# audeering/opensmile

Measured on NVIDIA H100. Metric: LLD frames/sec (16kHz, 25ms/10ms), higher is better.
Workload: dtype f32

## Files before the change

opensmile_b200/csrc/lld_common.cuh:

```cuda
#pragma once
#include <cstdio>

#include "fft_radix.cuh"
#include "kernels.cuh"

namespace osm {

struct SmemLayout {
  int zbuf, samp, raw, rawPcm, mbar, winLut, tw, splitTw, melCoef, melRange, dctCos, dctLift, eql, melS, ring;
  int total;
  int sampFloats, rawPcmBytes;
};

__host__ __device__ inline int align_up(int x, int a) { return (x + a - 1) / a * a; }

constexpr int kLeadFrames = 8;

__host__ __device__ inline SmemLayout make_layout(const LldParams &p, int M, int F)
{
  SmemLayout L;
  int o = 0;
  L.zbuf = o; o += M * F * 8;
  const int S = p.frameStep + p.sPad;
  L.sampFloats = align_up((F - 1) * S + p.frameSize + ((p.frameSize - 1) / p.frameStep) * p.sPad + 2, 4);
  L.samp = o; o += L.sampFloats * 4;
  L.raw = o; o += F * 4;
  o = align_up(o, 16);
  L.rawPcmBytes = align_up(16 + (kLeadFrames + (F - 1) * p.frameStep + p.frameSize) * p.nChan * 2, 16);
  L.rawPcm = o; o += L.rawPcmBytes;
  L.mbar = o; o += 16;
  L.winLut = o; o += M * 16;
  L.tw = o; o += p.twCount * 8;
  L.splitTw = o; o += (M / 2 + 1) * 8;
  o = align_up(o, 16);
  L.melCoef = o; o += (p.melVCount + 4) * 8;
  L.melRange = o; o += 2 * (p.nBands + 2) * 4;
  o = align_up(o, 16);
  L.dctCos = o; o += max(p.dctRows * p.dctStride, p.opKind == 0 ? p.nBands * 16 : 0) * 4;
  L.dctLift = o; o += p.nStat * 4;
  L.eql = o; o += (p.opKind == 1 ? p.nBands : 0) * 4;
  o = align_up(o, 16);
  if (L.sampFloats >= p.nBands * F) L.melS = L.samp;
  else { L.melS = o; o += p.nBands * F * 4; }
  L.ring = o; o += p.nStat * 2 * F * 4;
  L.total = align_up(o, 16);
  return L;
}

__device__ __forceinline__ float div32767(float x)
{
  const float rc = 3.0518509447574615e-05f;
  const float q0 = __fmul_rn(x, rc);
  const float r = __fmaf_rn(-q0, 32767.0f, x);
  return __fmaf_rn(r, rc, q0);
}

#define OSM_COLD __noinline__
template <bool F32>
__device__ __forceinline__ float pcm_to_float_generic(const int16_t *s, int nChan)
{
  if constexpr (F32) return *reinterpret_cast<const float *>(s);
  float tmp = (float)s[0];
  for (int c = 1; c < nChan; c++) tmp = __fadd_rn(tmp, (float)s[c]);
  if (nChan == 1) return div32767(tmp);
  if (nChan == 2) return div32767(tmp * 0.5f);
  return __fdiv_rn(__fdiv_rn(tmp, (float)nChan), 32767.0f);
}
template <bool F32>
static __device__ OSM_COLD float pcm_to_float_slow(const int16_t *s, int nChan) { return pcm_to_float_generic<F32>(s, nChan); }

__device__ __forceinline__ uint32_t smem_u32(const void *p) { return (uint32_t)__cvta_generic_to_shared(p); }

__device__ __forceinline__ void mbar_init(uint64_t *bar, int count)
{
  asm volatile("mbarrier.init.shared::cta.b64 [%0], %1;" ::"r"(smem_u32(bar)), "r"(count));
  asm volatile("fence.mbarrier_init.release.cluster;" ::: "memory");
}
__device__ __forceinline__ void mbar_expect_tx(uint64_t *bar, uint32_t bytes)
{
  asm volatile("mbarrier.arrive.expect_tx.shared::cta.b64 _, [%0], %1;" ::"r"(smem_u32(bar)), "r"(bytes) : "memory");
}
__device__ __forceinline__ void bulk_g2s(void *dst, const void *src, uint32_t bytes, uint64_t *bar)
{
  asm volatile("cp.async.bulk.shared::cluster.global.mbarrier::complete_tx::bytes [%0], [%1], %2, [%3];"
               ::"r"(smem_u32(dst)), "l"(src), "r"(bytes), "r"(smem_u32(bar)) : "memory");
}
__device__ __forceinline__ void mbar_wait(uint64_t *bar, uint32_t parity)
{
  asm volatile(
      "{\n"
      ".reg .pred p;\n"
      "LAB_WAIT:\n"
      "mbarrier.try_wait.parity.shared::cta.b64 p, [%0], %1;\n"
      "@p bra LAB_DONE;\n"
      "bra LAB_WAIT;\n"
      "LAB_DONE:\n"
      "}\n" ::"r"(smem_u32(bar)), "r"(parity) : "memory");
}

struct ChunkCtx {
  int utt, a, b;
  int T;
  int s0;
  int sEnd;
  int nT;
  int tile0;
  long long uo;
  long long row0;
};

template <int F>
__device__ __forceinline__ ChunkCtx load_chunk(const LldParams &p, int chunk)
{
  ChunkCtx c;
  const ChunkRef cr = p.chunks[chunk];
  c.utt = cr.utt; c.a = cr.a; c.b = cr.b; c.tile0 = cr.tile0;
  c.uo = p.uttOff[cr.utt];
  const long long Ls = p.uttOff[cr.utt + 1] - c.uo;
  c.T = (int)((Ls - p.frameSize) / p.frameStep + 1);
  c.s0 = max(cr.a - p.halo, 0);
  c.sEnd = min(cr.b + p.halo, c.T);
  c.nT = (c.sEnd - c.s0 + F - 1) / F;
  c.row0 = p.rowOff[cr.utt];
  return c;
}

__device__ __forceinline__ int chunk_run_begin(const LldParams &p, int g)
{
  const long long w = (long long)p.chunks[0].w0 + (long long)g * p.ctaTiles;
  int lo = 0, hi = p.nChunks;
  while (lo < hi) {
    const int mid = (lo + hi) >> 1;
    if (p.chunks[mid].w0 < w) lo = mid + 1;
    else hi = mid;
  }
  return lo;
}

struct TileGeom {
  int fs;
  int nf;
  int count;
  int lead;
  int mis;
  uint32_t bytes;
  const char *src;
};

template <int F>
__device__ __forceinline__ TileGeom tile_geom(const LldParams &p, const ChunkCtx &c, int j)
{
  TileGeom g;
  g.fs = c.s0 + j * F;
  g.nf = min(F, c.sEnd - g.fs);
  const long long s0 = (long long)g.fs * p.frameStep;
  g.count = (g.nf - 1) * p.frameStep + p.frameSize;
  g.lead = (s0 > 0) ? kLeadFrames : 0;
  const char *a = reinterpret_cast<const char *>(p.pcm + (c.uo + s0 - g.lead) * p.nChan);
  g.mis = (int)(reinterpret_cast<uintptr_t>(a) & 15);
  g.src = a - g.mis;
  g.bytes = (uint32_t)align_up(g.mis + (g.lead + g.count) * p.nChan * 2, 16);
  return g;
}

__device__ __forceinline__ float div_exact(float x, float d, float rcp)
{
  const float ax = fabsf(x);
  if (rcp != 0.f && ax > 1e-30f && ax < 1e30f) {
    const float q0 = __fmul_rn(x, rcp);
    const float r = __fmaf_rn(-q0, d, x);
    return __fmaf_rn(r, rcp, q0);
  }
  return __fdiv_rn(x, d);
}

__device__ __forceinline__ int win_navail(int t, int n0, int c0, int Tprev)
{
  return (t < c0) ? Tprev : min(n0 + (t - c0) + 1, Tprev);
}

template <int M, int F, int NVW, int R, int MS, bool FIRST, bool LAST, bool VEC2>
__device__ __forceinline__ void fft_stage(float2 *__restrict__ Z, const float *__restrict__ sampF,
                                          const float *__restrict__ raw,
                                          const float4 *__restrict__ winLut,
                                          const float2 *__restrict__ tw,
                                          const LldParams &p, int vw, int f)
{
  constexpr int stride = MS / R;
  for (int t = vw; t < M / R; t += NVW) {
    const int blk = t / stride, j = t % stride;
    const int base = blk * MS + j;
    float2 v[R];
    if (FIRST) {
#pragma unroll
      for (int r = 0; r < R; r++) {
        const float4 wl = winLut[base + stride * r];
        const int off = __float_as_int(wl.z);
        float2 x;
        if (VEC2) {
          x = *reinterpret_cast<const float2 *>(sampF + off);
        } else {
          x.x = sampF[off];
          x.y = sampF[off + 1];
        }
        v[r] = make_float2(__fmul_rn(x.x, wl.x), __fmul_rn(x.y, wl.y));
      }
      if (base == 0 && p.preemph)
        v[0].x = __fmul_rn(__fmul_rn(p.oneMinusK, raw[f]), winLut[0].x);
      if (p.hasWinOffset) {
#pragma unroll
        for (int r = 0; r < R; r++) {
          const float nv = winLut[base + stride * r].w;
          if (nv >= 1.f) v[r].x = __fadd_rn(v[r].x, p.winOffset);
          if (nv >= 2.f) v[r].y = __fadd_rn(v[r].y, p.winOffset);
        }
      }
    } else {
#pragma unroll
      for (int r = 0; r < R; r++) v[r] = Z[(base + stride * r) * F + f];
    }
    Dft<R>::run(v);
    if (!LAST) {
      const float2 *twj = tw + j * R;
#pragma unroll
      for (int q = 1; q < R; q++) v[Dft<R>::out(q)] = cmul(v[Dft<R>::out(q)], twj[q]);
    }
#pragma unroll
    for (int q = 0; q < R; q++) Z[(base + stride * q) * F + f] = v[Dft<R>::out(q)];
  }
}

constexpr int kMaxLp = 8;

template <int F, int NVW>
__device__ __forceinline__ void plp_backend(const LldParams &p, const float *melS, const float *sCos,
                                            const float *sLift, float *acfS, float *dst, int vw, int f)
{
  const int nB = p.nBands, nFreq = p.plpNFreq, nAuto = p.plpNAuto;
  if (!p.plpIDFT) {
    for (int i = vw; i < nB; i += NVW) dst[i * (2 * F) + f] = melS[i * F + f];
    return;
  }
  for (int i = vw; i < nAuto; i += NVW) {
    const float *ct = sCos + i * p.dctStride;
    double tmp = 0.0;
    if (p.plpHtk) tmp = (double)ct[0] * (double)melS[f];
    for (int m = 1; m < nFreq - 1; m++) tmp = __dadd_rn(tmp, (double)ct[m] * (double)melS[(m - 1) * F + f]);
    tmp = __dadd_rn(tmp, (double)ct[nFreq - 1] * (double)melS[(nFreq - 3) * F + f]);
    const float a = (float)(tmp / (2.0 * (double)(nFreq - 1)));
    if (!p.plpLP) dst[i * (2 * F) + f] = a;
    else acfS[i * F + f] = a;
  }
  if (!p.plpLP) return;
  __syncthreads();
  if (vw == 0) {
    const int P = p.plpOrder;
    float r[kMaxLp + 1], a[kMaxLp], cc[kMaxLp + 1];
#pragma unroll
    for (int i = 0; i <= kMaxLp; i++) r[i] = (i <= P) ? acfS[i * F + f] : 0.f;
#pragma unroll
    for (int i = 0; i < kMaxLp; i++) a[i] = 0.f;
    float gain = 0.f;
    if (r[0] != 0.f) {
      float e = r[0];
#pragma unroll
      for (int m = 1; m <= kMaxLp; m++) {
        if (m <= P && e != 0.f) {
          float sum = r[m];
#pragma unroll
          for (int i = 1; i < m; i++) sum = __fadd_rn(sum, __fmul_rn(a[i - 1], r[m - i]));
          const float km = __fmul_rn(__fdiv_rn(-1.0f, e), sum);
          a[m - 1] = km;
#pragma unroll
          for (int i = 1; i <= m / 2; i++) {
            const float x = a[i - 1];
            a[i - 1] = __fadd_rn(a[i - 1], __fmul_rn(km, a[m - i - 1]));
            if ((i < (m / 2)) || ((m & 1) == 1)) a[m - i - 1] = __fadd_rn(a[m - i - 1], __fmul_rn(km, x));
          }
          e = __fmul_rn(e, __fsub_rn(1.0f, __fmul_rn(km, km)));
        }
      }
      gain = e;
    }
    if (!p.plpCeps) {
#pragma unroll
      for (int i = 0; i < kMaxLp; i++) if (i < P) dst[i * (2 * F) + f] = a[i];
      return;
    }
    if (gain <= 0.f) gain = 1.0f;
    int first = p.plpFirstCC < 1 ? 1 : p.plpFirstCC;
    const int last = p.plpLastCC > P ? P : p.plpLastCC;
#pragma unroll
    for (int n = 1; n <= kMaxLp; n++) {
      if (n >= first && n <= last) {
        double sum = 0.0;
#pragma unroll
        for (int i = 1; i < n; i++)
          sum = __dadd_rn(sum, (double)__fmul_rn(__fmul_rn((float)(n - i), a[i - 1]), cc[n - i - 1]));
        cc[n - first] = -__fadd_rn(a[n - first], (float)(sum / (double)n));
      }
    }
    const float zeroth = (float)(-log(1.0 / (double)gain));
    const int nC = p.nStat;
#pragma unroll
    for (int i = 0; i <= kMaxLp; i++) {
      if (i < nC) {
        float v;
        if (p.plpFirstCC == 0) {
          if (p.plpHtk) v = (i == nC - 1) ? zeroth : cc[i];
          else v = (i == 0) ? zeroth : cc[i - 1];
        } else {
          v = cc[i];
        }
        if (p.plpLifter) v = __fmul_rn(v, sLift[i]);
        dst[i * (2 * F) + f] = v;
      }
    }
  }
}

template <int F, int NT>
__device__ __forceinline__ void emit_interior(const float *__restrict__ ring, float *__restrict__ Dbuf,
                                              float *__restrict__ outS, int K, int dRows, int slot0, int rslot0,
                                              float norm1, float rcp1, float norm2, float rcp2, int tid)
{
  const int K3 = 3 * K;
  constexpr int DR = F + 4;
  for (int item = tid; item < K * DR; item += NT) {
    const int c = item / DR, tt = item - c * DR;
    const float *rc = ring + c * (2 * F);
    const int sl = slot0 + tt;
    const float dA = __fsub_rn(rc[(sl + 1) & (2 * F - 1)], rc[(sl - 1) & (2 * F - 1)]);
    const float dB = __fsub_rn(rc[(sl + 2) & (2 * F - 1)], rc[(sl - 2) & (2 * F - 1)]);
    const float dv = div_exact(__fadd_rn(dA, __fmul_rn(2.0f, dB)), norm1, rcp1);
    Dbuf[c * dRows + tt] = dv;
    const int rr = tt - 2;
    if (rr >= 0 && rr < F) outS[rr * K3 + K + c] = dv;
  }
  for (int item = tid; item < K * F; item += NT) {
    const int c = item / F, rr = item - c * F;
    outS[rr * K3 + c] = ring[c * (2 * F) + ((rslot0 + rr) & (2 * F - 1))];
  }
  __syncthreads();
  for (int item = tid; item < K * F; item += NT) {
    const int c = item / F, rr = item - c * F;
    const float *dt = Dbuf + c * dRows + rr + 2;
    const float dA = __fsub_rn(dt[1], dt[-1]);
    const float dB = __fsub_rn(dt[2], dt[-2]);
    outS[rr * K3 + 2 * K + c] = div_exact(__fadd_rn(dA, __fmul_rn(2.0f, dB)), norm2, rcp2);
  }
  __syncthreads();
}

template <int F, int NW>
__device__ OSM_COLD void emit_edge(const float *__restrict__ ring, float *__restrict__ Dbuf, float *__restrict__ outS,
                               int K, int W1, int W2, int T, int T1, int c01, int c02, int s0, int r0, int r1,
                               int d0, int d1, int dRows, float norm1, float rcp1, float norm2, float rcp2,
                               int warp, int lane)
{
  const int K3 = 3 * K, nr = r1 - r0;
  for (int c = warp; c < K; c += NW) {
    const float *rc = ring + c * (2 * F);
    for (int tt = lane; tt < d1 - d0; tt += 32) {
      const int t = d0 + tt;
      float num = 0.f;
      for (int i = 1; i <= W1; i++) {
        const int hi = t + i, lo = t - i;
        float later, prior;
        if (t - W1 < 0) {
          later = (hi >= T) ? 0.f : rc[(hi - s0) & (2 * F - 1)];
          prior = rc[(max(lo, 0) - s0) & (2 * F - 1)];
        } else {
          later = rc[(min(hi, T - 1) - s0) & (2 * F - 1)];
          prior = rc[(min(lo, T - 1) - s0) & (2 * F - 1)];
        }
        num = __fadd_rn(num, __fmul_rn((float)i, __fsub_rn(later, prior)));
      }
      const float dv = div_exact(num, norm1, rcp1);
      Dbuf[c * dRows + tt] = dv;
      if (t >= r0 && t < r1) outS[(t - r0) * K3 + K + c] = dv;
    }
    for (int rr = lane; rr < nr; rr += 32) outS[rr * K3 + c] = rc[(r0 + rr - s0) & (2 * F - 1)];
  }
  __syncthreads();
  for (int c = warp; c < K; c += NW) {
    const float *dc = Dbuf + c * dRows - d0;
    for (int rr = lane; rr < nr; rr += 32) {
      const int t = r0 + rr;
      const int navail2 = win_navail(t, c01, c02, T1);
      float num = 0.f;
      for (int i = 1; i <= W2; i++) {
        const int hi = t + i, lo = t - i;
        float later, prior;
        if (t - W2 < 0) {
          later = (hi >= navail2) ? 0.f : dc[hi];
          prior = dc[max(lo, 0)];
        } else {
          later = dc[min(hi, navail2 - 1)];
          prior = dc[min(lo, navail2 - 1)];
        }
        num = __fadd_rn(num, __fmul_rn((float)i, __fsub_rn(later, prior)));
      }
      outS[rr * K3 + 2 * K + c] = div_exact(num, norm2, rcp2);
    }
  }
  __syncthreads();
}

}
```

opensmile_b200/csrc/lld_fast.cu:

```cuda
#include "lld_common.cuh"

namespace osm {

enum { kPhStage, kPhPass1, kPhPass2, kPhMel, kPhDct, kPhEmit, kPhStore, kPhKernel, kPhKernelMax, kPhTiles, kPhSlots };
#ifdef OSM_LLD_PHASE_CLOCKS
__device__ unsigned long long gLld512Phase[kPhSlots];
#define OSM_PHASE(k)                                                    \
  do {                                                                  \
    if (tid == 0) {                                                     \
      const long long c_ = clock64();                                   \
      sPh[k] += (unsigned long long)(c_ - phT);                         \
      phT = c_;                                                         \
    }                                                                   \
  } while (0)
#else
#define OSM_PHASE(k) do {} while (0)
#endif

namespace {

constexpr int kM = 256, kF = 32, kNT = 256, kNW = 8;
constexpr int kKMax = 16;
constexpr int kPartOff = 9216;

__device__ __forceinline__ void dft4_d0(float2 &a, float2 &b, float2 &c, float2 &d)
{
  const float2 t0 = cadd(a, c), t1 = csub(a, c), bb = b;
  a = cadd(t0, bb);
  c = csub(t0, bb);
  b = make_float2(t1.x + bb.y, t1.y - bb.x);
  d = make_float2(t1.x - bb.y, t1.y + bb.x);
}

template <int NZR>
__device__ __forceinline__ void dft16_first(float2 (&v)[16])
{
  dft4(v[0], v[4], v[8], v[12]);
  if (NZR <= 13) {
    dft4_d0(v[1], v[5], v[9], v[13]);
    dft4_d0(v[2], v[6], v[10], v[14]);
    dft4_d0(v[3], v[7], v[11], v[15]);
  } else {
    dft4(v[1], v[5], v[9], v[13]);
    dft4(v[2], v[6], v[10], v[14]);
    dft4(v[3], v[7], v[11], v[15]);
  }
  const float c1 = 0.92387953251128675613f, s1 = 0.38268343236508977173f;
  const float c2 = 0.70710678118654752440f;
  v[5] = cmul(v[5], make_float2(c1, -s1));
  { float2 a = v[6]; v[6] = make_float2(c2 * (a.x + a.y), c2 * (a.y - a.x)); }
  v[7] = cmul(v[7], make_float2(s1, -c1));
  { float2 a = v[9]; v[9] = make_float2(c2 * (a.x + a.y), c2 * (a.y - a.x)); }
  v[10] = cmul_mi(v[10]);
  { float2 a = v[11]; v[11] = make_float2(c2 * (a.y - a.x), -c2 * (a.x + a.y)); }
  v[13] = cmul(v[13], make_float2(s1, -c1));
  { float2 a = v[14]; v[14] = make_float2(c2 * (a.y - a.x), -c2 * (a.x + a.y)); }
  v[15] = cmul(v[15], make_float2(-c1, s1));
#pragma unroll
  for (int k1 = 0; k1 < 4; k1++) dft4(v[4 * k1], v[4 * k1 + 1], v[4 * k1 + 2], v[4 * k1 + 3]);
}

__device__ __forceinline__ void split_pair(float2 a, float2 b, float2 w, float &pk, float &pm)
{
  const float2 e2 = make_float2(a.x + b.x, a.y - b.y);
  const float2 o2 = make_float2(a.x - b.x, a.y + b.y);
  const float2 t2 = cmul(o2, w);
  const float xr = e2.x + t2.y, xi = e2.y - t2.x;
  const float yr = e2.x - t2.y, yi = e2.y + t2.x;
  pk = __fmaf_rn(xr, xr, __fmul_rn(xi, xi));
  pm = __fmaf_rn(yr, yr, __fmul_rn(yi, yi));
}

template <int NZR>
__global__ void __launch_bounds__(kNT, 2) lld512_kernel(const LldParams p)
{
  constexpr int M = kM, F = kF, NT = kNT, NW = kNW;
  using D16 = Dft<16>;

  extern __shared__ __align__(16) unsigned char smem[];
  __shared__ ChunkCtx sCx[2];
  __shared__ int sRun[2];
  const SmemLayout L = make_layout(p, M, F);
  float2 *Z = reinterpret_cast<float2 *>(smem + L.zbuf);
  float *P = reinterpret_cast<float *>(smem + L.zbuf);
  float *samp = reinterpret_cast<float *>(smem + L.samp);
  float *raw = reinterpret_cast<float *>(smem + L.raw);
  unsigned char *rawPcm = smem + L.rawPcm;
  uint64_t *mbar = reinterpret_cast<uint64_t *>(smem + L.mbar);
  float4 *sWinLut = reinterpret_cast<float4 *>(smem + L.winLut);
  float2 *sTw = reinterpret_cast<float2 *>(smem + L.tw);
  float2 *sSplit = reinterpret_cast<float2 *>(smem + L.splitTw);
  float2 *sMelCoef = reinterpret_cast<float2 *>(smem + L.melCoef);
  int *sMelRange = reinterpret_cast<int *>(smem + L.melRange);
  float *sDct = reinterpret_cast<float *>(smem + L.dctCos);
  float *sLift = reinterpret_cast<float *>(smem + L.dctLift);
  float *ring = reinterpret_cast<float *>(smem + L.ring);
  float *Dbuf = reinterpret_cast<float *>(smem + L.zbuf);

  const int tid = threadIdx.x;
  const int warp = tid >> 5, f = tid & 31;

  if (tid == 0) mbar_init(mbar, 1);
  if (tid < 2) sRun[tid] = chunk_run_begin(p, blockIdx.x + tid);
  for (int i = tid; i < M; i += NT) sWinLut[i] = p.winLut[i];
  for (int i = tid; i < p.twCount; i += NT) sTw[i] = p.twiddles[i];
  for (int i = tid; i < M / 2 + 1; i += NT) sSplit[i] = p.splitTw[i];
  for (int i = tid; i < p.melVCount; i += NT) sMelCoef[i] = p.melVisit[i];
  for (int i = tid; i < p.nBands + 2; i += NT) { sMelRange[i] = p.melRange[i]; sMelRange[p.nBands + 2 + i] = p.melVB[i]; }
  for (int i = tid; i < p.nBands * kKMax; i += NT) {
    const int m = i / kKMax, c = i - m * kKMax;
    sDct[i] = (c < p.nStat) ? p.dctCos[c * p.dctStride + m] : 0.f;
  }
  for (int i = tid; i < p.nStat; i += NT) sLift[i] = p.dctLift[i];
  for (int i = tid; i < L.sampFloats; i += NT) samp[i] = 0.f;
  for (int i = tid; i < F; i += NT) raw[i] = 0.f;
  __syncthreads();

  const int hop = p.frameStep;
  const int S = hop + p.sPad;
  uint32_t phase = 0;
#ifdef OSM_LLD_PHASE_CLOCKS
  __shared__ unsigned long long sPh[kPhSlots];
  if (tid < kPhSlots) sPh[tid] = 0;
  const long long phT0 = clock64();
  long long phT = phT0;
#endif

  int chunk = sRun[0];
  const int chunkEnd = sRun[1];
  if (chunk >= chunkEnd) return;
  int cpar = 0;
  if (tid == 0) {
    sCx[0] = load_chunk<F>(p, chunk);
    const TileGeom g0 = tile_geom<F>(p, sCx[0], 0);
    mbar_expect_tx(mbar, g0.bytes);
    bulk_g2s(rawPcm, g0.src, g0.bytes, mbar);
  }
  __syncthreads();
  int j = 0;
  int emitted = sCx[0].a;

  const int tA = (warp == 0) ? 0 : warp, tB = (warp == 0) ? 8 : 16 - warp;
  const int wl = (warp == 0) ? 8 : warp, wh = (warp == 0) ? 0 : warp;
  const int melBs = p.melSplit[warp], melBe = p.melSplit[warp + 1];

  while (chunk < chunkEnd) {
    const ChunkCtx &cx = sCx[cpar];

    mbar_wait(mbar, phase);
    phase ^= 1;
    {
      const TileGeom tg = tile_geom<F>(p, cx, j);
      const int count = tg.count;
      const int16_t *rp = reinterpret_cast<const int16_t *>(rawPcm + tg.mis) + tg.lead;
      const bool aligned = (tg.mis == 0);
      const bool hasLead = tg.lead > 0;
      const float ks = p.preDe ? p.preK : -p.preK;
#pragma unroll 1
      for (int i = tid * 8; i < count; i += NT * 8) {
        int wds[4];
        if (aligned) {
          const int4 w4 = *reinterpret_cast<const int4 *>(rp + i);
          wds[0] = w4.x; wds[1] = w4.y; wds[2] = w4.z; wds[3] = w4.w;
        } else {
          const unsigned short *up = reinterpret_cast<const unsigned short *>(rp + i);
#pragma unroll
          for (int jj = 0; jj < 4; jj++) wds[jj] = (int)((unsigned)up[2 * jj] | ((unsigned)up[2 * jj + 1] << 16));
        }
        float x[8], y[8];
#pragma unroll
        for (int jj = 0; jj < 4; jj++) {
          x[2 * jj] = div32767((float)(short)(wds[jj] & 0xffff));
          x[2 * jj + 1] = div32767((float)(wds[jj] >> 16));
        }
        if (p.preemph) {
          float xprev = 0.f;
          if (i > 0 || hasLead) xprev = div32767((float)rp[i - 1]);
#pragma unroll
          for (int jj = 0; jj < 8; jj++) y[jj] = __fadd_rn(x[jj], __fmul_rn(ks, (jj == 0) ? xprev : x[jj - 1]));
        } else {
#pragma unroll
          for (int jj = 0; jj < 8; jj++) y[jj] = x[jj];
        }
        const int q = (int)__umulhi((unsigned)i, p.hopMagic);
        float *dst = samp + i + q * p.sPad;
        if (i == q * hop && q < F) raw[q] = x[0];
#pragma unroll
        for (int jj = 0; jj < 8; jj += 2) *reinterpret_cast<float2 *>(dst + jj) = make_float2(y[jj], y[jj + 1]);
      }
    }
    __syncthreads();
    if (tid == 0) {
      if (j + 1 < cx.nT) {
        const TileGeom gn = tile_geom<F>(p, cx, j + 1);
        mbar_expect_tx(mbar, gn.bytes);
        bulk_g2s(rawPcm, gn.src, gn.bytes, mbar);
      } else if (chunk + 1 < chunkEnd) {
        const ChunkCtx cn = load_chunk<F>(p, chunk + 1);
        sCx[cpar ^ 1] = cn;
        const TileGeom gn = tile_geom<F>(p, cn, 0);
        mbar_expect_tx(mbar, gn.bytes);
        bulk_g2s(rawPcm, gn.src, gn.bytes, mbar);
      }
    }
    OSM_PHASE(kPhStage);

    {
      const float *sampF = samp + f * S;
      const float2 *tw0 = sTw + p.twOff[0];
#pragma unroll 1
      for (int t = warp; t < 16; t += NW) {
        float2 v[16];
#pragma unroll
        for (int r = 0; r < 16; r++) {
          if (r < NZR) {
            const float4 wl = sWinLut[t + 16 * r];
            const float2 x = *reinterpret_cast<const float2 *>(sampF + __float_as_int(wl.z));
            v[r] = make_float2(__fmul_rn(x.x, wl.x), __fmul_rn(x.y, wl.y));
          } else {
            v[r] = make_float2(0.f, 0.f);
          }
        }
        if (t == 0 && p.preemph)
          v[0].x = __fmul_rn(__fmul_rn(p.oneMinusK, raw[f]), sWinLut[0].x);
        dft16_first<NZR>(v);
        const float2 *twj = tw0 + t * 16;
#pragma unroll
        for (int q = 1; q < 16; q++) v[D16::out(q)] = cmul(v[D16::out(q)], twj[q]);
        float2 *zp = Z + t * F + f;
#pragma unroll
        for (int q = 0; q < 16; q++) zp[(16 * q) * F] = v[D16::out(q)];
      }
    }
    __syncthreads();
    OSM_PHASE(kPhPass1);

    {
      float2 A[16], v[16];
#pragma unroll 2
      for (int h = 0; h < 2; h++) {
        const float2 *zp = Z + ((h ? tB : tA) * 16) * F + f;
#pragma unroll
        for (int r = 0; r < 16; r++) v[r] = zp[r * F];
        D16::run(v);
        if (h == 0) {
#pragma unroll
          for (int r = 0; r < 16; r++) A[r] = v[r];
        }
      }
      const float2 x0 = A[D16::out(0)];
      if (warp == 0) {
        float2 na[8], nb[8];
#pragma unroll
        for (int q = 0; q < 8; q++) { na[q] = v[D16::out(q)]; nb[q] = A[D16::out(q + 1)]; }
#pragma unroll
        for (int q = 0; q < 8; q++) { A[D16::out(q)] = na[q]; v[D16::out(q)] = nb[q]; }
      }
      float pk[16], pm[16];
      {
        const float2 *swl = sSplit + wl, *swh = sSplit + (256 - wh);
#pragma unroll
        for (int q = 0; q < 16; q++) {
          const float2 aq = A[D16::out(q)], bq = v[D16::out(15 - q)];
          if (q < 8) split_pair(aq, bq, swl[16 * q], pk[q], pm[q]);
          else       split_pair(bq, aq, swh[-16 * q], pk[q], pm[q]);
        }
      }
      __syncthreads();
      {
        float *Plo = P + wl * F + f, *Plm = P + (256 - wl) * F + f;
        float *Phi = P + (256 - wh) * F + f, *Phm = P + wh * F + f;
#pragma unroll
        for (int q = 0; q < 8; q++) { Plo[(16 * q) * F] = pk[q]; Plm[(-16 * q) * F] = pm[q]; }
#pragma unroll
        for (int q = 8; q < 16; q++) {
          Phi[(-16 * q) * F] = pk[q];
          if (q > 8 || warp != 0) Phm[(16 * q) * F] = pm[q];
        }
      }
      if (warp == 0) {
        const float xr = 2.0f * (x0.x + x0.y), yr = 2.0f * (x0.x - x0.y);
        P[f] = __fmul_rn(xr, xr);
        P[M * F + f] = __fmul_rn(yr, yr);
      }
    }
    __syncthreads();
    OSM_PHASE(kPhPass2);

    float *melS = P + kPartOff;
    if (melBs < melBe) {
      const int *sVB = sMelRange + p.nBands + 2;
      float cur = 0.f;
      for (int r = melBs; r <= melBe; r++) {
        float nxt = 0.f;
        const float *pp = P + sMelRange[r] * F + f;
        const int v0 = sVB[r];
        const float4 *cp = reinterpret_cast<const float4 *>(sMelCoef + v0);
#pragma unroll 1
        for (int q = (sVB[r + 1] - v0) >> 2; q > 0; q--, pp += 4 * F, cp += 2) {
          const float p0 = pp[0], p1 = pp[F], p2 = pp[2 * F], p3 = pp[3 * F];
          const float4 wa = cp[0], wb = cp[1];
          cur = __fmaf_rn(p0, wa.x, cur); nxt = __fmaf_rn(p0, wa.y, nxt);
          cur = __fmaf_rn(p1, wa.z, cur); nxt = __fmaf_rn(p1, wa.w, nxt);
          cur = __fmaf_rn(p2, wb.x, cur); nxt = __fmaf_rn(p2, wb.y, nxt);
          cur = __fmaf_rn(p3, wb.z, cur); nxt = __fmaf_rn(p3, wb.w, nxt);
        }
        if (r > melBs) {
          float mval = __fmul_rn(cur, p.melScale);
          if (p.doLog) mval = (mval < p.melfloor) ? p.logMelfloor : logf(mval);
          melS[(r - 1) * F + f] = mval;
        }
        cur = nxt;
      }
    }
    __syncthreads();
    OSM_PHASE(kPhMel);

    const int ringBase = (j & 1) * F;
    {
      const int i = 2 * warp;
      if (i < p.nStat) {
        const float2 *cc = reinterpret_cast<const float2 *>(sDct + i);
        const float *lp = melS + f;
        float a0 = 0.f, a1 = 0.f;
#pragma unroll 4
        for (int m = 0; m < p.nBands; m++, lp += F, cc += kKMax / 2) {
          const float l0 = lp[0];
          const float2 c = cc[0];
          a0 = __fmaf_rn(l0, c.x, a0); a1 = __fmaf_rn(l0, c.y, a1);
        }
        ring[i * (2 * F) + ringBase + f] = __fmul_rn(a0, sLift[i]);
        if (i + 1 < p.nStat) ring[(i + 1) * (2 * F) + ringBase + f] = __fmul_rn(a1, sLift[i + 1]);
      }
    }
    __syncthreads();
    OSM_PHASE(kPhDct);

    const int tfs = cx.s0 + j * F;
    if (!p.fused) {
      const int tot = min(F, cx.sEnd - tfs) * p.nStat;
      for (int idx = tid; idx < tot; idx += NT) {
        const int ff = idx / p.nStat, c = idx - ff * p.nStat;
        p.out[(cx.row0 + tfs + ff) * p.outStride + p.outCol + c] = ring[c * (2 * F) + ringBase + ff];
      }
    } else {
      const int K = p.nStat, W1 = p.fW1, W2 = p.fW2, H = W1 + W2;
      const int T = cx.T;
      const int r0 = emitted;
      const int r1 = (j + 1 == cx.nT) ? cx.b : min(tfs + F - H, cx.b);
      const int T1 = T + W1, c01 = max(T - W1, 0), c02 = max(c01 - W2, 0);
      const float norm1 = p.fNorm1, norm2 = p.fNorm2;
      const int d0 = max(r0 - W2, 0), d1 = min(r1 + W2, T1);
      const int dRows = F + 24;
      float *outS = Dbuf + ((K * dRows + 3) & ~3);
      const int K3 = 3 * K;
      const int nr = r1 - r0;
      const bool interior1 = (d0 >= W1) && (d1 + W1 <= T);
      const bool interior2 = (r0 >= W2) && (r1 <= c02);
      if (interior1 && interior2 && W1 == 2 && W2 == 2 && nr == F) {
        emit_interior<F, NT>(ring, Dbuf, outS, K, dRows, d0 - cx.s0, r0 - cx.s0, norm1, p.fRcp1, norm2, p.fRcp2, tid);
      } else {
        emit_edge<F, NW>(ring, Dbuf, outS, K, W1, W2, T, T1, c01, c02, cx.s0, r0, r1, d0, d1, dRows, norm1, p.fRcp1, norm2, p.fRcp2, warp, f);
      }
      OSM_PHASE(kPhEmit);
      {
        float *o = p.out + (cx.row0 + r0) * (long long)K3;
        const int n = nr * K3;
        for (int i = tid; i < n; i += NT) o[i] = outS[i];
      }
      emitted = r1;
    }
    OSM_PHASE(kPhStore);
#ifdef OSM_LLD_PHASE_CLOCKS
    if (tid == 0) sPh[kPhTiles]++;
#endif

    j++;
    if (j == cx.nT) {
      chunk++;
      j = 0;
      cpar ^= 1;
      if (chunk < chunkEnd) emitted = sCx[cpar].a;
    }
  }
#ifdef OSM_LLD_PHASE_CLOCKS
  if (tid == 0) {
    sPh[kPhKernel] = (unsigned long long)(clock64() - phT0);
    for (int k = 0; k < kPhSlots; k++)
      if (k != kPhKernelMax) atomicAdd(&gLld512Phase[k], sPh[k]);
    atomicMax(&gLld512Phase[kPhKernelMax], sPh[kPhKernel]);
  }
#endif
}

template <int NZR>
cudaError_t launch_fast_t(const LldParams &p, int numSMs, cudaStream_t st, LldLaunchInfo *info, bool launch)
{
  const size_t smem = (size_t)make_layout(p, kM, kF).total;
  auto kern = lld512_kernel<NZR>;
  cudaError_t e = cudaFuncSetAttribute(kern, cudaFuncAttributeMaxDynamicSharedMemorySize, (int)smem);
  if (e != cudaSuccess) return e;
  int occ = 0;
  e = cudaOccupancyMaxActiveBlocksPerMultiprocessor(&occ, kern, kNT, smem);
  if (e != cudaSuccess) return e;
  if (occ < 1) return cudaErrorLaunchOutOfResources;
  const int grid = launch ? p.nRuns : numSMs * occ;
  if (info) {
    info->grid = grid; info->block = kNT; info->smem = smem; info->nChunks = p.nChunks;
    info->kernel = NZR == 13 ? "lld512_kernel<13>" : "lld512_kernel<16>";
  }
  if (!launch) return cudaSuccess;
  kern<<<grid, kNT, smem, st>>>(p);
  return cudaGetLastError();
}

}

bool lld_fast_applies(const LldParams &p, int nfft)
{
  return nfft == 512 && !p.narrow && p.opKind == 0 && p.magOut == nullptr && p.melUsePower && p.nChan == 1 &&
         p.frameStep % 8 == 0 && p.frameSize % 8 == 0 && p.frameSize <= 512 && !p.hasWinOffset && p.nStat <= kKMax &&
         ((p.frameStep + p.sPad) % 2) == 0;
}

cudaError_t launch_lld_fast(const LldParams &p, int numSMs, cudaStream_t st, LldLaunchInfo *info, bool launch)
{
  if (p.frameSize <= 416) return launch_fast_t<13>(p, numSMs, st, info, launch);
  return launch_fast_t<16>(p, numSMs, st, info, launch);
}

#ifdef OSM_LLD_PHASE_CLOCKS
extern "C" __attribute__((visibility("default"))) int osm_b200_lld512_phase_clocks(unsigned long long *out)
{
  cudaError_t e = cudaMemcpyFromSymbol(out, gLld512Phase, sizeof(gLld512Phase));
  if (e == cudaSuccess) {
    static const unsigned long long zero[kPhSlots] = {};
    e = cudaMemcpyToSymbol(gLld512Phase, zero, sizeof(zero));
  }
  return (int)e;
}
#endif

}
```

Measured before the change: 935.6 million.

## Specialize PCM staging, add warp-per-channel delta emit, vectorize output store

PCM staging gets a fast path for the common aligned, lead-present, pre-emphasis case. Its frame index and destination pointer are now updated incrementally instead of recomputed with a multiply-high each iteration. The interior delta emit is rewritten so each warp handles one channel with lanes as rows, and the divide slow path becomes warp-uniform via __any_sync. The output tile's shared staging buffer is shifted to match global alignment, so the store uses float4 writes with scalar head and tail. This adds code complexity and relies on K ≤ 16 channels and F == 32 for the warp mapping.

```diff
diff --git a/opensmile_b200/csrc/lld_common.cuh b/opensmile_b200/csrc/lld_common.cuh
--- a/opensmile_b200/csrc/lld_common.cuh
+++ b/opensmile_b200/csrc/lld_common.cuh
@@ -174,6 +174,17 @@
   return __fdiv_rn(x, d);
 }
 
+__device__ __forceinline__ float div_exact_warp(float x, float d, float rcp, bool live = true)
+{
+  const float q0 = __fmul_rn(x, rcp);
+  const float r = __fmaf_rn(-q0, d, x);
+  float y = __fmaf_rn(r, rcp, q0);
+  const float ax = fabsf(x);
+  const bool slow = live && !(rcp != 0.f && ax > 1e-30f && ax < 1e30f);
+  if (__any_sync(0xffffffffu, slow) && slow) y = __fdiv_rn(x, d);
+  return y;
+}
+
 __device__ __forceinline__ int win_navail(int t, int n0, int c0, int Tprev)
 {
   return (t < c0) ? Tprev : min(n0 + (t - c0) + 1, Tprev);
@@ -348,6 +359,57 @@
     const float dA = __fsub_rn(dt[1], dt[-1]);
     const float dB = __fsub_rn(dt[2], dt[-2]);
     outS[rr * K3 + 2 * K + c] = div_exact(__fadd_rn(dA, __fmul_rn(2.0f, dB)), norm2, rcp2);
+  }
+  __syncthreads();
+}
+
+template <int F, int NW>
+__device__ __forceinline__ void emit_interior_w2(const float *__restrict__ ring, float *__restrict__ Dbuf,
+                                                 float *__restrict__ outS, int K, int dRows, int slot0, int rslot0,
+                                                 float norm1, float rcp1, float norm2, float rcp2, int warp, int lane)
+{
+  static_assert(F == 32, "lane = row");
+  constexpr int RM = 2 * F - 1;
+  const int K3 = 3 * K;
+  const int sm = slot0 + lane, sh = slot0 + F + (lane & 3);
+  const int m2 = (sm - 2) & RM, m1 = (sm - 1) & RM, p1 = (sm + 1) & RM, p2 = (sm + 2) & RM;
+  const int h2 = (sh - 2) & RM, h1 = (sh - 1) & RM, g1 = (sh + 1) & RM, g2 = (sh + 2) & RM;
+  const int rs = (rslot0 + lane) & RM;
+#pragma unroll
+  for (int u = 0; u < 2; u++) {
+    const int c = warp + NW * u;
+    if (c < K) {
+      const float *rc = ring + c * (2 * F);
+      const float dA = __fsub_rn(rc[p1], rc[m1]);
+      const float dB = __fsub_rn(rc[p2], rc[m2]);
+      const float dv = div_exact_warp(__fadd_rn(dA, __fmul_rn(2.0f, dB)), norm1, rcp1);
+      Dbuf[c * dRows + lane] = dv;
+      if (lane >= 2) outS[(lane - 2) * K3 + K + c] = dv;
+      outS[lane * K3 + c] = rc[rs];
+    }
+  }
+  {
+    const int ch = warp + NW * (lane >> 2);
+    const bool live = ch < K;
+    const float *rc = ring + (live ? ch : 0) * (2 * F);
+    const float dA = __fsub_rn(rc[g1], rc[h1]);
+    const float dB = __fsub_rn(rc[g2], rc[h2]);
+    const float dv = div_exact_warp(__fadd_rn(dA, __fmul_rn(2.0f, dB)), norm1, rcp1, live);
+    if (live) {
+      Dbuf[ch * dRows + F + (lane & 3)] = dv;
+      if ((lane & 3) < 2) outS[(F - 2 + (lane & 3)) * K3 + K + ch] = dv;
+    }
+  }
+  __syncthreads();
+#pragma unroll
+  for (int u = 0; u < 2; u++) {
+    const int c = warp + NW * u;
+    if (c < K) {
+      const float *dt = Dbuf + c * dRows + lane + 2;
+      const float dA = __fsub_rn(dt[1], dt[-1]);
+      const float dB = __fsub_rn(dt[2], dt[-2]);
+      outS[lane * K3 + 2 * K + c] = div_exact_warp(__fadd_rn(dA, __fmul_rn(2.0f, dB)), norm2, rcp2);
+    }
   }
   __syncthreads();
 }
diff --git a/opensmile_b200/csrc/lld_fast.cu b/opensmile_b200/csrc/lld_fast.cu
--- a/opensmile_b200/csrc/lld_fast.cu
+++ b/opensmile_b200/csrc/lld_fast.cu
@@ -22,6 +22,27 @@
 constexpr int kM = 256, kF = 32, kNT = 256, kNW = 8;
 constexpr int kKMax = 16;
 constexpr int kPartOff = 9216;
+constexpr int kStageStep = kNT * 8;
+
+__device__ __forceinline__ float stage8(const int (&wds)[4], bool preemph, float xprev, float ks, float *dst)
+{
+  float x[8], y[8];
+#pragma unroll
+  for (int jj = 0; jj < 4; jj++) {
+    x[2 * jj] = div32767((float)(short)(wds[jj] & 0xffff));
+    x[2 * jj + 1] = div32767((float)(wds[jj] >> 16));
+  }
+  if (preemph) {
+#pragma unroll
+    for (int jj = 0; jj < 8; jj++) y[jj] = __fadd_rn(x[jj], __fmul_rn(ks, (jj == 0) ? xprev : x[jj - 1]));
+  } else {
+#pragma unroll
+    for (int jj = 0; jj < 8; jj++) y[jj] = x[jj];
+  }
+#pragma unroll
+  for (int jj = 0; jj < 8; jj += 2) *reinterpret_cast<float2 *>(dst + jj) = make_float2(y[jj], y[jj + 1]);
+  return x[0];
+}
 
 __device__ __forceinline__ void dft4_d0(float2 &a, float2 &b, float2 &c, float2 &d)
 {
@@ -118,6 +139,8 @@
 
   const int hop = p.frameStep;
   const int S = hop + p.sPad;
+  const int stageQ = kStageStep / hop, stageRem = kStageStep - stageQ * hop;
+  const int stageDst = kStageStep + stageQ * p.sPad;
   uint32_t phase = 0;
 #ifdef OSM_LLD_PHASE_CLOCKS
   __shared__ unsigned long long sPh[kPhSlots];
@@ -153,40 +176,41 @@
       const TileGeom tg = tile_geom<F>(p, cx, j);
       const int count = tg.count;
       const int16_t *rp = reinterpret_cast<const int16_t *>(rawPcm + tg.mis) + tg.lead;
-      const bool aligned = (tg.mis == 0);
-      const bool hasLead = tg.lead > 0;
       const float ks = p.preDe ? p.preK : -p.preK;
+      int i = tid * 8;
+      int q = (int)__umulhi((unsigned)i, p.hopMagic);
+      int rem = i - q * hop;
+      float *dst = samp + i + q * p.sPad;
+      if (tg.mis == 0 && tg.lead > 0 && p.preemph) {
 #pragma unroll 1
-      for (int i = tid * 8; i < count; i += NT * 8) {
-        int wds[4];
-        if (aligned) {
+        for (; i < count; i += kStageStep) {
           const int4 w4 = *reinterpret_cast<const int4 *>(rp + i);
-          wds[0] = w4.x; wds[1] = w4.y; wds[2] = w4.z; wds[3] = w4.w;
-        } else {
-          const unsigned short *up = reinterpret_cast<const unsigned short *>(rp + i);
-#pragma unroll
-          for (int jj = 0; jj < 4; jj++) wds[jj] = (int)((unsigned)up[2 * jj] | ((unsigned)up[2 * jj + 1] << 16));
-        }
-        float x[8], y[8];
-#pragma unroll
-        for (int jj = 0; jj < 4; jj++) {
-          x[2 * jj] = div32767((float)(short)(wds[jj] & 0xffff));
-          x[2 * jj + 1] = div32767((float)(wds[jj] >> 16));
-        }
-        if (p.preemph) {
-          float xprev = 0.f;
-          if (i > 0 || hasLead) xprev = div32767((float)rp[i - 1]);
-#pragma unroll
-          for (int jj = 0; jj < 8; jj++) y[jj] = __fadd_rn(x[jj], __fmul_rn(ks, (jj == 0) ? xprev : x[jj - 1]));
-        } else {
-#pragma unroll
-          for (int jj = 0; jj < 8; jj++) y[jj] = x[jj];
-        }
-        const int q = (int)__umulhi((unsigned)i, p.hopMagic);
-        float *dst = samp + i + q * p.sPad;
-        if (i == q * hop && q < F) raw[q] = x[0];
-#pragma unroll
-        for (int jj = 0; jj < 8; jj += 2) *reinterpret_cast<float2 *>(dst + jj) = make_float2(y[jj], y[jj + 1]);
+          const int wds[4] = {w4.x, w4.y, w4.z, w4.w};
+          const float x0 = stage8(wds, true, div32767((float)rp[i - 1]), ks, dst);
+          if (rem == 0 && q < F) raw[q] = x0;
+          rem += stageRem; q += stageQ; dst += stageDst;
+          if (rem >= hop) { rem -= hop; q++; dst += p.sPad; }
+        }
+      } else {
+        const bool aligned = (tg.mis == 0);
+        const bool hasLead = tg.lead > 0;
+#pragma unroll 1
+        for (; i < count; i += kStageStep) {
+          int wds[4];
+          if (aligned) {
+            const int4 w4 = *reinterpret_cast<const int4 *>(rp + i);
+            wds[0] = w4.x; wds[1] = w4.y; wds[2] = w4.z; wds[3] = w4.w;
+          } else {
+            const unsigned short *up = reinterpret_cast<const unsigned short *>(rp + i);
+#pragma unroll
+            for (int jj = 0; jj < 4; jj++) wds[jj] = (int)((unsigned)up[2 * jj] | ((unsigned)up[2 * jj + 1] << 16));
+          }
+          const float xprev = (p.preemph && (i > 0 || hasLead)) ? div32767((float)rp[i - 1]) : 0.f;
+          const float x0 = stage8(wds, p.preemph, xprev, ks, dst);
+          if (rem == 0 && q < F) raw[q] = x0;
+          rem += stageRem; q += stageQ; dst += stageDst;
+          if (rem >= hop) { rem -= hop; q++; dst += p.sPad; }
+        }
       }
     }
     __syncthreads();
@@ -352,21 +376,29 @@
       const float norm1 = p.fNorm1, norm2 = p.fNorm2;
       const int d0 = max(r0 - W2, 0), d1 = min(r1 + W2, T1);
       const int dRows = F + 24;
-      float *outS = Dbuf + ((K * dRows + 3) & ~3);
       const int K3 = 3 * K;
+      float *o = p.out + (cx.row0 + r0) * (long long)K3;
+      const int sh = (int)((reinterpret_cast<uintptr_t>(o) >> 2) & 3);
+      float *outS = Dbuf + ((K * dRows + 3) & ~3) + sh;
       const int nr = r1 - r0;
       const bool interior1 = (d0 >= W1) && (d1 + W1 <= T);
       const bool interior2 = (r0 >= W2) && (r1 <= c02);
       if (interior1 && interior2 && W1 == 2 && W2 == 2 && nr == F) {
-        emit_interior<F, NT>(ring, Dbuf, outS, K, dRows, d0 - cx.s0, r0 - cx.s0, norm1, p.fRcp1, norm2, p.fRcp2, tid);
+        emit_interior_w2<F, NW>(ring, Dbuf, outS, K, dRows, d0 - cx.s0, r0 - cx.s0, norm1, p.fRcp1, norm2, p.fRcp2, warp, f);
       } else {
         emit_edge<F, NW>(ring, Dbuf, outS, K, W1, W2, T, T1, c01, c02, cx.s0, r0, r1, d0, d1, dRows, norm1, p.fRcp1, norm2, p.fRcp2, warp, f);
       }
       OSM_PHASE(kPhEmit);
       {
-        float *o = p.out + (cx.row0 + r0) * (long long)K3;
         const int n = nr * K3;
-        for (int i = tid; i < n; i += NT) o[i] = outS[i];
+        const int hd = min((4 - sh) & 3, n);
+        const int nv = (n - hd) >> 2;
+        const float4 *s4 = reinterpret_cast<const float4 *>(outS + hd);
+        float4 *o4 = reinterpret_cast<float4 *>(o + hd);
+        for (int i = tid; i < nv; i += NT) o4[i] = s4[i];
+        const int tl = hd + 4 * nv, ti = tid - (NT - 32);
+        if (tid < hd) o[tid] = outS[tid];
+        if (ti >= 0 && ti < n - tl) o[tl + ti] = outS[tl + ti];
       }
       emitted = r1;
     }
```

After: 957.7 million, median of 6. 1.02x the previous value.
